# ishine/zerovox.cpp

Hardware: AMD Instinct MI355X
Metric: audio-seconds/wall-second (xRT) end-to-end phoneme->22.05 kHz wav (higher is better)
Workload: dtype f16*f16->f32 (MFMA) convs, f32 (MFMA) attention/linear, f32 activations

## Files before the change

### zerovox.cpp_amd/csrc/capi.cpp

```cpp
#include <algorithm>
#include <cmath>
#include <cstring>
#include <map>
#include <optional>
#include <string>
#include <thread>
#include <vector>

#include "common.h"
#include "model.h"
#include "knobs.h"

using zv::Model;

struct PendingBatch;
struct zv_model
{
    Model        *m;
    PendingBatch *pending;
};

static void free_pending(zv_model *m);
static void lane0_select(zv_model *m);
static void use_lane0(zv_model *m);
// ... 278 lines not shown
static zv_status run_single(zv_model *m, const Request &r, std::optional<Taps> taps = std::nullopt)
{
    return guarded([&] {
        check_request(m, r);
        Model &M = *m->m;
        use_lane0(m);
        const uint32_t n = r.n[0], T = r.T[0];
        const bool tg = r.targets(), pc = r.phoneme_controls() || tg, dur = r.timings();
        const size_t E = M.E(), b_ids = (size_t)n * 4, b_hid = (size_t)T * E * 4, b_wav = (size_t)T * M.hp.audio_hop_size * 4;
        const size_t b_ctl = r.prosody || tg ? zv::CTL_STRIDE * 4 : 0, b_pctl = pc ? (size_t)n * zv::PCTL_STRIDE * 4 : 0;
        if (!taps) M.reserve(n, T);
        Layout L;
        const size_t o_nf = L.at(4), o_ids = L.at(b_ids), o_pun = L.at(b_ids), o_sty = L.at(E * 4), o_ctl = L.at(b_ctl),
                     o_pctl = L.at(b_pctl), o_hid = L.at(b_hid);
        const size_t o_mel = taps ? 0 : L.at((size_t)T * M.hp.audio_num_mels * 4), o_wav = taps ? 0 : L.at(b_wav),
                     o_cum = taps ? 0 : L.at(dur ? b_ids : 0), o_live = L.at(r.fitted && !taps ? sizeof(zv::Seg) : 0);
        char *io = (char *)M.io_scratch(L.size());
        int32_t *d_nf = (int32_t *)(io + o_nf), *d_ids = (int32_t *)(io + o_ids), *d_pun = (int32_t *)(io + o_pun);
        float *d_sty = (float *)(io + o_sty), *d_hid = (float *)(io + o_hid);
        std::vector<float> ctl(b_ctl / 4), pctl(b_pctl / 4);
        std::vector<int32_t> cum(dur ? n : 0);
        pack_controls(r, ctl.data(), pctl.data());
        zv::Batch bt = zv::Batch::single(n, T, r.num_phonemes[0]);
        bt.has_targets = tg;
        ZV_HIP(hipMemcpyAsync(d_ids, r.ids[0], b_ids, hipMemcpyHostToDevice, M.stream()));
        ZV_HIP(hipMemcpyAsync(d_pun, r.puncts[0], b_ids, hipMemcpyHostToDevice, M.stream()));
        ZV_HIP(hipMemcpyAsync(d_sty, r.styles[0], E * 4, hipMemcpyHostToDevice, M.stream()));
        if (b_ctl)
        {
            bt.d_ctl = (const float *)(io + o_ctl);
            ZV_HIP(hipMemcpyAsync(io + o_ctl, ctl.data(), b_ctl, hipMemcpyHostToDevice, M.stream()));
        }
        if (b_pctl)
        {
            bt.d_pctl = (const float *)(io + o_pctl);
            ZV_HIP(hipMemcpyAsync(io + o_pctl, pctl.data(), b_pctl, hipMemcpyHostToDevice, M.stream()));
        }
        int32_t nf = 0;
        if (taps)
// ... 1 lines not shown
            const Model::EncoderTaps t = M.encode_dev(bt, d_ids, d_pun, d_sty, d_hid, d_nf);
            ZV_HIP(hipMemcpyAsync(r.out[0], d_hid, b_hid, hipMemcpyDeviceToHost, M.stream()));
            ZV_HIP(hipMemcpyAsync(&nf, d_nf, 4, hipMemcpyDeviceToHost, M.stream()));
            if (taps->features) ZV_HIP(hipMemcpyAsync(taps->features, t.features, (size_t)n * E * 4, hipMemcpyDeviceToHost, M.stream()));
            if (taps->logdur) ZV_HIP(hipMemcpyAsync(taps->logdur, t.logdur, b_ids, hipMemcpyDeviceToHost, M.stream()));
            if (taps->pitch) ZV_HIP(hipMemcpyAsync(taps->pitch, t.pitch, b_ids, hipMemcpyDeviceToHost, M.stream()));
            if (taps->energy) ZV_HIP(hipMemcpyAsync(taps->energy, t.energy, b_ids, hipMemcpyDeviceToHost, M.stream()));
            if (taps->pitch_bucket) ZV_HIP(hipMemcpyAsync(taps->pitch_bucket, t.pitch_bucket, b_ids, hipMemcpyDeviceToHost, M.stream()));
            if (taps->energy_bucket) ZV_HIP(hipMemcpyAsync(taps->energy_bucket, t.energy_bucket, b_ids, hipMemcpyDeviceToHost, M.stream()));
            if (dur) ZV_HIP(hipMemcpyAsync(cum.data(), t.cum, b_ids, hipMemcpyDeviceToHost, M.stream()));
        }
        else
        {
            float *d_mel = (float *)(io + o_mel), *d_wav = (float *)(io + o_wav);
            if (dur) bt.d_cum = (int32_t *)(io + o_cum);
            if (r.fitted) bt.d_frm_live = (zv::Seg *)(io + o_live);
            M.chain_dev(bt, d_ids, d_pun, d_sty, d_hid, d_mel, d_wav, d_nf);
            ZV_HIP(hipMemcpyAsync(&nf, d_nf, 4, hipMemcpyDeviceToHost, M.stream()));
            if (dur) ZV_HIP(hipMemcpyAsync(cum.data(), bt.d_cum, b_ids, hipMemcpyDeviceToHost, M.stream()));
            ZV_HIP(hipMemcpyAsync(r.out[0], d_wav, b_wav, hipMemcpyDeviceToHost, M.stream()));
        }
        M.sync();
        if (r.n_frames) r.n_frames[0] = (uint32_t)nf;
        if (dur) durations_from_cum(cum.data(), 1, r.n, r.T, r.durations);
    });
}

zv_status zv_encode_taps(zv_model *m, const int32_t *ids, const int32_t *puncts, const float *style, uint32_t n,
                         uint32_t num_phonemes, uint32_t T, float *hidden, uint32_t *n_frames, float *features, float *logdur,
                         float *pitch, float *energy, int32_t *pitch_bucket, int32_t *energy_bucket)
{
// ... 223 lines not shown
    zv::Batch bt;
    bt.nseg = (int)r.count;
    bt.n_max = zv::round_up((int)nmax, 32);
    bt.n_real = (int)nmax;
    bt.t_max = zv::round_up((int)tmax, 64);
    bt.n_rows = (size_t)bt.nseg * bt.n_max;
    bt.t_rows = (size_t)bt.nseg * bt.t_max;
    Layout in;
    const size_t b_tab = (size_t)(bt.nseg + 1) * sizeof(zv::Seg);
    const size_t i_tok = in.at(b_tab), i_frm = in.at(b_tab), i_ids = in.at(bt.n_rows * 4), i_pun = in.at(bt.n_rows * 4),
                 i_sty = in.at((size_t)bt.nseg * E * 4), i_ctl = in.at(ctl ? (size_t)bt.nseg * zv::CTL_STRIDE * 4 : 0),
                 i_pctl = in.at(pc ? bt.n_rows * zv::PCTL_STRIDE * 4 : 0), b_in = in.size();
    Layout dev;
    const size_t o_nf = dev.at((size_t)bt.nseg * 4), o_in = dev.at(b_in), o_hid = dev.at(bt.t_rows * E * 4),
                 o_mel = dev.at(bt.t_rows * Mm * 4), o_wav = dev.at(bt.t_rows * hop * 4), o_cum = dev.at(dur ? bt.n_rows * 4 : 0),
                 o_live = dev.at(r.fitted ? (size_t)bt.nseg * sizeof(zv::Seg) : 0);
    M.reserve_batch(bt);
    char *io = (char *)M.io_scratch(dev.size());
    size_t wav_bytes = 0;
    pb.woff.assign(r.count, 0);
    for (uint32_t u = 0; u < r.count; u++)
    {
        pb.woff[u] = wav_bytes;
        wav_bytes += (size_t)r.T[u] * hop * 4;
    }
    Layout host;
    const size_t p_in = host.at(b_in), p_nf = host.at((size_t)bt.nseg * 4), p_wav = host.at(wav_bytes),
                 p_cum = host.at(dur ? bt.n_rows * 4 : 0);
    char *pin = (char *)M.pinned_scratch(host.size());
    char *d_in = io + o_in, *h_in = pin + p_in;
    {
// ... 11 lines not shown
            memcpy(h_sty + (size_t)u * E, r.styles[u], E * 4);
            n0 += n;
            t0 += t;
        }
        h_tok[r.count] = zv::Seg{0, n0, n0, 0};
        h_frm[r.count] = zv::Seg{0, t0, 0, 0};
        pack_controls(r, (float *)(h_in + i_ctl), (float *)(h_in + i_pctl));
    }
    bt.d_tok = (const zv::Seg *)(d_in + i_tok);
    bt.d_frm = (const zv::Seg *)(d_in + i_frm);
    if (ctl) bt.d_ctl = (const float *)(d_in + i_ctl);
    bt.has_targets = tg;
    if (pc) bt.d_pctl = (const float *)(d_in + i_pctl);
    if (dur) bt.d_cum = (int32_t *)(io + o_cum);
    if (r.fitted) bt.d_frm_live = (zv::Seg *)(io + o_live);
    int32_t *d_nf = (int32_t *)(io + o_nf), *d_ids = (int32_t *)(d_in + i_ids), *d_pun = (int32_t *)(d_in + i_pun);
    float *d_sty = (float *)(d_in + i_sty), *d_hid = (float *)(io + o_hid), *d_mel = (float *)(io + o_mel), *d_wav = (float *)(io + o_wav);
    int32_t *h_nf = (int32_t *)(pin + p_nf), *h_cum = dur ? (int32_t *)(pin + p_cum) : nullptr;
    char *h_wav = pin + p_wav;
    const int G = (M.tail_groups() > 1 && bt.nseg >= 4 && wav_bytes >= ((size_t)16 << 20) && !M.profiling && M.dbg_layer.kind < 0)
                      ? std::min(M.tail_groups(), (int)bt.nseg / 2) : 1;
    try
    {
        hipStream_t cs = M.copy_stream();
        pb.gb.assign(G + 1, r.count);
        pb.gb[0] = 0;
        const uint64_t seq = M.next_batch_seq();
        ZV_HIP(hipEventRecord(M.batch_event(seq, 0), M.stream()));
        if (G <= 1)
        {
// ... 605 lines not shown
```

### zerovox.cpp_amd/csrc/decoder.cpp

```cpp
#include "schedule.h"

#include <cmath>

namespace zv
{

Model::DecLayout Model::dec_layout(DeviceArena &a, const Batch &bt) const
{
    const size_t S = (size_t)bt.nseg, L = bt.t_rows, B = 2 * E(), R = (size_t)dec_.R, CAT = B + R;
    DecLayout d{(bt.t_max + 31) / 32, round_up(dec_.fc_out + 64, 64), 2 * (int)CAT + 64};
    d.h = a.take_n<float>(S * d.hs);
    for (float **st : {&d.st_x, &d.st_t, &d.st_y, &d.st_a}) *st = a.take_n<float>(S * d.ss);
    for (double **p : {&d.part_t, &d.part_o}) *p = a.take_n<double>(S * d.nblk * CAT * 2);
    d.cat = a.take_n<float>(L * CAT);
    for (float **x : {&d.t1, &d.sc, &d.x0, &d.xa}) *x = a.take_n<float>(L * B);
    d.asr_t = a.take_n<float>(L * R);
    d.xa16 = a.take_n<_Float16>(L * CAT);
    d.t16 = a.take_n<_Float16>(L * B);
    d.xr16 = a.take_n<_Float16>(L * CAT);
    return d;
}

void Model::decode_dev(const Batch &bt, const float *d_hidden, const float *d_styles, float *d_mel)
{
    if (bt.t_rows == 0 || bt.t_max <= 0) fail(ZV_ERR_ARG, "T must be > 0");
    const DecLayout lay = dec_layout(stage_arena(bt), bt);
    const Segs fr = bt.frames();
    const int Ed = (int)E(), B = 2 * Ed, R = dec_.R, CAT = B + R, S = bt.nseg;
    const size_t L = bt.t_rows;
    const int nblk = lay.nblk, hs = lay.hs, ss = lay.ss;
    float *const h = lay.h, *const st_x = lay.st_x, *const st_t = lay.st_t, *const st_y = lay.st_y, *const st_a = lay.st_a;
    double *const part_t = lay.part_t, *const part_o = lay.part_o;
    float *const cat = lay.cat, *const t1 = lay.t1, *const sc = lay.sc, *const x0 = lay.x0, *const xa = lay.xa, *const asr_t = lay.asr_t;
    _Float16 *const xa16 = lay.xa16, *const t16 = lay.t16, *const xr16 = lay.xr16;
    const double Ld = (double)L;
    const int pre_env = knob(ZV_DEC_PREPASS);
    const bool prepass = pre_env >= 0 ? pre_env != 0 : (size_t)bt.t_max * bt.nseg >= 256;

    ZV_LAUNCH("dec_adain_fc", 4.0 * dec_.fc_out * (Ed + 2), 2.0 * S * dec_.fc_out * Ed,
              launch_linear(stream(), d_styles, Ed, Ed, dec_.fcW, dec_.fcB, dec_.fc_out, h, hs, dec_.fcExtra, segs_single(S)));

    const float rsqrt2 = (float)(1.0 / sqrt(2.0));

    auto finalize = [&](const double *part, int C, float *stat, int c_off) {
        ZV_LAUNCH("dec_in_stats", 16.0 * S * nblk * C, 4.0 * S * nblk * C,
                  launch_stats_finalize(stream(), part, nblk, C, 1e-5f, stat, ss, c_off, fr, 1));
    };
    auto norm_input = [&](ConvJob &j, const float *x, int ldx, int C, const double *part, int Cpart, float *stat, const float *g,
                          const float *b, int gb_seg, _Float16 *op16, _Float16 *raw16 = nullptr) {
        if (prepass)
        {
            ZV_LAUNCH("dec_norm_operand", 6.0 * Ld * C, 8.0 * Ld * C,
                      launch_norm_act_f16(stream(), x, ldx, C, part, nblk, Cpart, 1e-5f, stat, ss, g, b, gb_seg, 0.2f, op16, C, fr, raw16));
            j.x0 = op16;
            j.ldx = C;
            j.pro = PRO_RAW_F16;
        }
        else
        {
            finalize(part, Cpart, stat, 0);
            j.x0 = x;
            j.ldx = ldx;
            j.pro = PRO_NORM_ACT;
            j.pstat = stat;
            j.pstat_seg = ss;
            j.pa = g;
            j.pb = b;
            j.pab_seg = gb_seg;
// ... 119 lines not shown
    const int ldos[5] = {CAT, CAT, Ed, Ed, Ed};
    const int cparts[5] = {B, B, B, Ed, Ed};
    float *sts[5] = {st_x, st_x, st_x, st_y, st_y};
    for (int i = 0; i < 5; i++)
    {
        const DecBlk &b = dec_.dec[i];
        block(b, cur, ldc, cparts[i], sts[i], h + b.g1, h + b.g1 + b.cin, h + b.g2, h + b.g2 + b.cout, hs, outs[i], ldos[i], i < 4);
        cur = outs[i];
        ldc = ldos[i];
    }
    if (dbg_layer.done) return;
    {
        ConvJob j = job(dec_.to_out);
        j.x0 = cur;
        j.ldx = ldc;
        j.out = d_mel;
        j.ldo = dec_.M;
        if (dbg_layer.kind == ZV_LAYER_DEC_TO_OUT) dbg_inject(const_cast<float *>(cur), ldc, Ed, L);
        conv(&j, 1, fr, 1, "dec_conv", conv_bytes(Ld, Ed, dec_.M, 1, false), conv_flops(Ld, Ed, dec_.M, 1));
        if (dbg_layer.kind == ZV_LAYER_DEC_TO_OUT) dbg_extract(d_mel, dec_.M, dec_.M, L);
    }
}

}
```

### zerovox.cpp_amd/csrc/encoder.cpp

```cpp
#include "schedule.h"

#include <cmath>

namespace zv
{

Model::EncLayout Model::enc_layout(DeviceArena &a, const Batch &bt) const
{
    const size_t n = bt.n_rows, Ed = E();
    EncLayout e{round_up(enc_.dur.V, 16)};
    for (float **p : {&e.x, &e.y}) *p = a.take_n<float>(n * Ed);
    e.qkv = a.take_n<float>(n * 3 * Ed);
    for (float **p : {&e.o, &e.f}) *p = a.take_n<float>(n * Ed);
    e.hh = a.take_n<_Float16>(n * round_up(hp.conv_filter_size, 16));
    for (float **p : {&e.va, &e.vb}) *p = a.take_n<float>(n * e.Vp);
    for (float **p : {&e.t.logdur, &e.t.pitch, &e.t.energy}) *p = a.take_n<float>(n);
    for (int32_t **p : {&e.t.pitch_bucket, &e.t.energy_bucket}) *p = a.take_n<int32_t>(n);
    e.t.cum = bt.d_cum ? bt.d_cum : a.take_n<int32_t>(n);
    e.t.features = e.x;
    return e;
}

Model::EncoderTaps Model::encode_dev(const Batch &bt, const int32_t *d_ids, const int32_t *d_puncts, const float *d_styles,
                                     float *d_hidden, int32_t *d_nframes)
// ... 113 lines not shown
    };
    predictor(enc_.dur, t.logdur, nullptr, nullptr, 0, 0);
    predictor(enc_.pitch, t.pitch, enc_.pitch_emb, t.pitch_bucket, CTL_PITCH, PCTL_PITCH);
    if (dbg_layer.done) return t;
    predictor(enc_.energy, t.energy, enc_.energy_emb, t.energy_bucket, CTL_ENERGY, PCTL_ENERGY);
    if (dbg_layer.done) return t;
    if (bt.has_targets)
    {
        if (!bt.d_ctl || !bt.d_pctl) fail(ZV_ERR_ARG, "a batch with target durations needs its control rows");
        ZV_LAUNCH("enc_fit_durations", 24.0 * nd, 0.0, launch_fit_durations(stream(), t.logdur, bt.d_ctl, bt.d_pctl, tk, fr));
    }
    ZV_LAUNCH("enc_length_regulator", 4.0 * (nd + (double)bt.t_rows) * Ed, 0.0,
              launch_length_regulator(stream(), x, Ed, t.logdur, Ed, d_hidden, Ed, t.cum, d_nframes, tk, fr, bt.d_ctl, bt.d_pctl));
    if (bt.d_frm_live)
        ZV_LAUNCH("enc_live_frames", 36.0 * bt.nseg, 0.0, launch_live_frames(stream(), d_nframes, bt.d_frm_live, fr));
    return t;
}

void Model::debug_layernorm(int index, uint32_t n)
{
    const int l = index >> 1, Ed = (int)E();
    if (index < 0 || l >= (int)enc_.layers.size()) return;
    const EncLayer &Ly = enc_.layers[l];
    float *d = (float *)io_scratch(2 * (size_t)n * Ed * 4), *y = d + (size_t)n * Ed;
    dbg_inject(d, Ed, Ed, n);
    ZV_HIP(launch_add_layernorm(stream(), d, Ed, nullptr, 0, Ed, Ed, (index & 1) ? Ly.ln2w : Ly.ln1w, (index & 1) ? Ly.ln2b : Ly.ln1b,
                                1e-5f, y, Ed, segs_single((int)n)));
    dbg_extract(y, Ed, Ed, n);
}

// ... 2 lines not shown
```

### zerovox.cpp_amd/csrc/kernels.h

```cpp
#pragma once

#include <hip/hip_runtime.h>
#include <stdint.h>

#ifdef ZV_DIAG
#define ZV_DBGBITS(x) (x)
#else
#define ZV_DBGBITS(x) 0
#endif

namespace zv
{

__host__ __device__ static inline int round_up(int x, int a) { return (x + a - 1) / a * a; }

struct Seg
{
    int32_t row0, rows;
    int32_t aux;
    int32_t pad;
};
struct Segs
{
    const Seg *tab;
// ... 161 lines not shown
{
    const float *x0, *x1, *x2;
    int          ldx, L, C, K;
    float        pscale, slope;
    const uint16_t *w;
    float        bias;
    float       *out;
    Segs         segs;
    int          rate;
    int          runs;
};
hipError_t launch_out_conv(hipStream_t s, const OutConvArgs &a);

hipError_t launch_stats_partial(hipStream_t s, const float *x, int ldx, int C, double *part, int nblk, const Segs &segs, int rate);
hipError_t launch_stats_finalize(hipStream_t s, const double *part, int nblk, int C, float eps, float *stat, int stat_seg,
                                 int c_off, const Segs &segs, int rate);
hipError_t launch_norm_apply(hipStream_t s, const float *x, int ldx, int C, const float *stat, int stat_seg, const float *g,
                             const float *b, float *y, int ldy, double *part, int nblk, const Segs &segs);

hipError_t launch_act_f16(hipStream_t s, const float *x0, const float *x1, const float *x2, float pscale, float slope, void *out, size_t n);
hipError_t launch_norm_act_f16(hipStream_t s, const float *x, int ldx, int C, const double *part, int nblk, int Cpart, float eps,
                               float *stat, int stat_seg, const float *ga, const float *be, int gb_seg, float slope, void *y,
                               int ldy, const Segs &segs, void *yraw = nullptr);

hipError_t launch_linear(hipStream_t s, const float *x, int ldx, int in, const float *W, const float *b, int out, float *y,
                         int ldy, const float *extra, const Segs &segs);

hipError_t launch_embed(hipStream_t s, const int32_t *ids, const int32_t *puncts, const float *wemb, int emb,
                        const float *pemb, int pdim, const float *posenc, float *x, int ld, const Segs &segs);
hipError_t launch_attention(hipStream_t s, const float *q, const float *k, const float *v, int ld, int H, int dk,
                            float inv_temp, float *o, int ldo, const Segs &segs);
constexpr int CTL_STRIDE = 8;
constexpr int CTL_DURATION = 0;
constexpr int CTL_PITCH = 1;
constexpr int CTL_ENERGY = 3;
constexpr int CTL_TARGET = 5;
constexpr int PCTL_STRIDE = 4;
constexpr int PCTL_FRAMES = 0;
// ... 17 lines not shown
hipError_t launch_length_regulator(hipStream_t s, const float *feat, int ld, const float *logdur, int C, float *hidden,
                                   int ldh, int32_t *cum, int32_t *n_frames, const Segs &tokens, const Segs &frames,
                                   const float *ctl = nullptr, const float *pctl = nullptr);

constexpr int FIT_MAX_TOKENS = 3584;
hipError_t launch_fit_durations(hipStream_t s, const float *logdur, const float *ctl, const float *pctl, const Segs &tokens,
                                const Segs &frames);

hipError_t launch_live_frames(hipStream_t s, const int32_t *n_frames, Seg *live, const Segs &frames);
hipError_t launch_zero_tail(hipStream_t s, float *x, int C, const Segs &frames, const Segs &live, int rate);

constexpr int VOC_RUN_MARGIN = 16;
hipError_t launch_voc_runs(hipStream_t s, const float *mel, int M, float *mel_c, int32_t *eq, Seg *runs, const Segs &frames, int H);
hipError_t launch_voc_run_fill(hipStream_t s, float *x, const Segs &runs, int rate);

}
```

### zerovox.cpp_amd/csrc/knobs.h

```cpp
#pragma once

namespace zv
{

#define ZV_KNOB_LIST(X)                                                                                                               \
    X(ZV_NO_FUSE, 0)                                                                  \
    X(ZV_NO_TRIPLE, 0)                                                                          \
    X(ZV_FUSE256, 0)                                                \
    X(ZV_NO_MERGE, 0)                                                               \
    X(ZV_MERGE_ALWAYS, 0)                 \
    X(ZV_MERGE_SEQ, 1)          \
    X(ZV_MERGE_MAXC, 256)                                  \
    X(ZV_TAIL_GROUPS, 8)                                                        \
    X(ZV_ARENA_FILL, 0)                                         \
    X(ZV_DEC_PREPASS, -1)                                      \
    X(ZV_CONV_MT, 0)                                                              \
    X(ZV_CONV_NT, 0)                                                     \
    X(ZV_CONV_SINGLE, 1)                                    \
    X(ZV_CONV_GEMM, 1)                  \
    X(ZV_CONV_STREAM, 1)        \
    X(ZV_VOC_RUNS, 1)           \
    X(ZV_UP_GEMM, 1)            \
    X(ZV_GEMM_ORDER, 2)         \
    X(ZV_PAIR_MT, 0)                                                                  \
    X(ZV_CONV_XCD, 1)           \
    X(ZV_CONV_WARM, 1)          \
    X(ZV_LINEAR_MERGED, 1)      \
    X(ZV_BLOCK64, 3)            \
    X(ZV_PAIR64_RING, 1)               \
    X(ZV_TRIPLE_V2, 1)                               \
    X(ZV_TRIPLE_DB, 1)                                                                     \
    X(ZV_TRIPLE_INTERLEAVE, 1)                                                               \
    X(ZV_ATT_SCALAR, 0)                                                                               \
    X(ZV_ATT_MFMA, 0)                                                          \
    X(ZV_LN_TAIL, 1)

// ... 34 lines not shown
```

### zerovox.cpp_amd/csrc/misc_kernels.hip

```cpp
#include "kernels.h"
#include "knobs.h"
#include "fit_durations.h"

#include <cstring>

namespace zv
{

__device__ __forceinline__ double wave_sum(double v)
{
#pragma unroll
    for (int o = 32; o > 0; o >>= 1) v += __shfl_xor(v, o, 64);
    return v;
}
__device__ __forceinline__ float wave_sum_f(float v)
{
#pragma unroll
    for (int o = 32; o > 0; o >>= 1) v += __shfl_xor(v, o, 64);
    return v;
}

typedef float floatx16m __attribute__((ext_vector_type(16)));

__global__ __launch_bounds__(256) void stats_partial_kernel(const float *__restrict__ x, int ldx, int C,
// ... 24 lines not shown
    {
        const double a = (red[0][0][cl] + red[0][1][cl]) + (red[0][2][cl] + red[0][3][cl]);
        const double b = (red[1][0][cl] + red[1][1][cl]) + (red[1][2][cl] + red[1][3][cl]);
        *(double2 *)(part + (((size_t)useg * nblk + blk) * C + c) * 2) = make_double2(a, b);
    }
}

hipError_t launch_stats_partial(hipStream_t s, const float *x, int ldx, int C, double *part, int nblk, const Segs &segs, int rate)
{
    const int nb = (segs.max_rows * rate + 31) / 32;
    if (nb > nblk || segs.nseg < 1) return hipErrorInvalidValue;
    hipLaunchKernelGGL(stats_partial_kernel, dim3((C + 63) / 64, nb, segs.nseg), dim3(256), 0, s, x, ldx, C, part, nblk, segs, rate);
    return hipGetLastError();
}

__device__ __forceinline__ float2 stats_from_partials(const double *__restrict__ p, int C, int nb, int L, float eps)
{
    double s1 = 0.0, s2 = 0.0;
    for (int b0 = 0; b0 < nb; b0 += 8)
    {
        double2 v[8];
#pragma unroll
        for (int i = 0; i < 8; i++) v[i] = *(const double2 *)(p + (size_t)(b0 + i < nb ? b0 + i : nb - 1) * C * 2);
#pragma unroll
        for (int i = 0; i < 8; i++)
            if (b0 + i < nb)
            {
                s1 += v[i].x;
                s2 += v[i].y;
            }
    }
    const double mean = s1 / (double)L;
    double var = s2 / (double)L - mean * mean;
    var = var > 0.0 ? var : 0.0;
    return make_float2((float)mean, 1.0f / sqrtf((float)var + eps));
}

__global__ __launch_bounds__(64) void stats_finalize_kernel(const double *__restrict__ part, int nblk, int C, float eps,
                                                            float *__restrict__ stat, int stat_seg, int c_off,
                                                            const Segs segs, int rate)
{
    const int useg = blockIdx.y;
    const Seg sg = seg_at(segs, useg);
    const int L = sg.rows * rate;
    const int c = blockIdx.x * 64 + threadIdx.x;
    if (c >= C || L <= 0) return;
    const float2 mr = stats_from_partials(part + ((size_t)useg * nblk * C + c) * 2, C, (L + 31) >> 5, L, eps);
    float *o = stat + (size_t)useg * stat_seg + 2 * (c_off + c);
    o[0] = mr.x;
    o[1] = mr.y;
}

hipError_t launch_stats_finalize(hipStream_t s, const double *part, int nblk, int C, float eps, float *stat, int stat_seg,
                                 int c_off, const Segs &segs, int rate)
{
    if (segs.nseg < 1) return hipErrorInvalidValue;
    hipLaunchKernelGGL(stats_finalize_kernel, dim3((C + 63) / 64, segs.nseg), dim3(64), 0, s, part, nblk, C, eps, stat, stat_seg,
                       c_off, segs, rate);
    return hipGetLastError();
}

__global__ __launch_bounds__(256) void norm_apply_kernel(const float *__restrict__ x, int ldx, int C,
                                                         const float *__restrict__ stat, int stat_seg,
                                                         const float *__restrict__ g, const float *__restrict__ b,
                                                         float *__restrict__ y, int ldy, double *__restrict__ part, int nblk,
                                                         const Segs segs)
{
    __shared__ double red[2][4][64];
    const int useg = blockIdx.z, blk = blockIdx.y;
    const Seg sg = seg_at(segs, useg);
    const int L = sg.rows;
    if (blk * 32 >= L) return;
    const int cl = threadIdx.x & 63, rg = threadIdx.x >> 6;
// ... 35 lines not shown
hipError_t launch_norm_apply(hipStream_t s, const float *x, int ldx, int C, const float *stat, int stat_seg, const float *g,
                             const float *b, float *y, int ldy, double *part, int nblk, const Segs &segs)
{
    const int nb = (segs.max_rows + 31) / 32;
    if ((part && nb > nblk) || segs.nseg < 1) return hipErrorInvalidValue;
    hipLaunchKernelGGL(norm_apply_kernel, dim3((C + 63) / 64, nb, segs.nseg), dim3(256), 0, s, x, ldx, C, stat, stat_seg, g, b, y,
                       ldy, part, nblk, segs);
    return hipGetLastError();
}

__global__ __launch_bounds__(256) void norm_act_f16_kernel(const float *__restrict__ x, int ldx, int C,
                                                           const double *__restrict__ part, int nblk, int Cpart, float eps,
                                                           float *__restrict__ stat, int stat_seg,
                                                           const float *__restrict__ ga, const float *__restrict__ be, int gb_seg,
                                                           float slope, _Float16 *__restrict__ y, int ldy, _Float16 *__restrict__ yraw,
                                                           const Segs segs)
{
    __shared__ float sm[4][64];
    const int useg = blockIdx.y;
    const Seg sg = seg_at(segs, useg);
    const int L = sg.rows;
    if (L <= 0) return;
    const int tid = threadIdx.x;
    if (tid < 64)
    {
        const int c = blockIdx.x * 64 + tid;
        float2 mr = make_float2(0.f, 0.f);
        float g = 0.f, b = 0.f;
        if (c < C)
        {
            float *st = stat + (size_t)useg * stat_seg + 2 * c;
            if (c < Cpart)
            {
                mr = stats_from_partials(part + ((size_t)useg * nblk * Cpart + c) * 2, Cpart, (L + 31) >> 5, L, eps);
                st[0] = mr.x;
                st[1] = mr.y;
            }
            else
                mr = make_float2(st[0], st[1]);
            g = ga[(size_t)useg * gb_seg + c];
            b = be[(size_t)useg * gb_seg + c];
        }
        sm[0][tid] = mr.x;
        sm[1][tid] = mr.y;
        sm[2][tid] = g;
        sm[3][tid] = b;
    }
    __syncthreads();
    const int c4 = (tid & 15) * 4, rl = tid >> 4;
// ... 33 lines not shown
            if (yr)
            {
                half4v hr;
                hr[0] = (_Float16)v[u].x;
                hr[1] = (_Float16)v[u].y;
                hr[2] = (_Float16)v[u].z;
                hr[3] = (_Float16)v[u].w;
                *(half4v *)(yr + (size_t)t * ldy) = hr;
            }
        }
    }
}

hipError_t launch_norm_act_f16(hipStream_t s, const float *x, int ldx, int C, const double *part, int nblk, int Cpart, float eps,
                               float *stat, int stat_seg, const float *ga, const float *be, int gb_seg, float slope, void *y,
                               int ldy, const Segs &segs, void *yraw)
{
    if ((C & 3) || (ldx & 3) || (ldy & 3) || segs.nseg < 1 || Cpart > C) return hipErrorInvalidValue;
    if (Cpart > 0 && (segs.max_rows + 31) / 32 > nblk) return hipErrorInvalidValue;
    int gz = 1;
    while (gz < 8 && (long)((C + 63) / 64) * segs.nseg * gz < 2048 && gz * 128 < segs.max_rows) gz <<= 1;
    hipLaunchKernelGGL(norm_act_f16_kernel, dim3((C + 63) / 64, segs.nseg, gz), dim3(256), 0, s, x, ldx, C, part, nblk, Cpart, eps, stat,
                       stat_seg, ga, be, gb_seg, slope, (_Float16 *)y, ldy, (_Float16 *)yraw, segs);
    return hipGetLastError();
}

typedef _Float16 half4v __attribute__((ext_vector_type(4)));
__global__ __launch_bounds__(256) void act_f16_kernel(const float4 *__restrict__ x0, const float4 *__restrict__ x1,
                                                      const float4 *__restrict__ x2, float pscale, float slope,
                                                      half4v *__restrict__ out, size_t n4)
{
    const size_t stride = (size_t)gridDim.x * 256;
    for (size_t i0 = (size_t)blockIdx.x * 256 + threadIdx.x; i0 < n4; i0 += 4 * stride)
    {
        float4 v[4], a[4], b[4];
#pragma unroll
        for (int u = 0; u < 4; u++)
        {
// ... 1248 lines not shown
    for (int k = 0; k < 4; k++)
    {
        const long i = i0 + k * 256 + threadIdx.x;
        if (i < n) dst[i] = src[i % rate];
    }
}

hipError_t launch_voc_run_fill(hipStream_t s, float *x, const Segs &runs, int rate)
{
    if (runs.nseg < 1 || runs.max_rows < 1 || rate < 1 || !runs.tab || !x) return hipErrorInvalidValue;
    const long per_seg = (long)runs.max_rows * rate;
    hipLaunchKernelGGL(voc_run_fill_kernel, dim3((unsigned)((per_seg + 1023) / 1024), runs.nseg), dim3(256), 0, s, x, runs.tab, rate);
    return hipGetLastError();
}

}
```

### zerovox.cpp_amd/csrc/model.h

```cpp
#pragma once

#include <cstdint>
#include <cstring>
#include <string>
#include <vector>

#include "common.h"
#include "gguf_reader.h"
#include "kernels.h"

namespace zv
{

struct ConvW
{
    void  *w = nullptr;
    void  *w8 = nullptr;
    float *bias = nullptr;
    int    K = 0, Cin = 0, Cout = 0, Cin_p = 0, Cout_p = 0, ck = 0;
};

struct DeviceArena
{
    char  *base = nullptr;
// ... 18 lines not shown
    int         launches;
};

struct Batch
{
    int        nseg = 1;
    int        n_max = 0, t_max = 0;
    int        n_real = 0;
    size_t     n_rows = 0, t_rows = 0;
    const Seg *d_tok = nullptr, *d_frm = nullptr;
    Seg        tok1{0, 0, 0, 0}, frm1{0, 0, 0, 0};
    const float *d_ctl = nullptr;
    const float *d_pctl = nullptr;
    int32_t *d_cum = nullptr;
    Seg *d_frm_live = nullptr;
    bool has_targets = false;

    static Batch single(uint32_t N, uint32_t T, uint32_t num_phonemes)
    {
        Batch b;
        b.n_max = (int)N;
        b.n_real = (int)N;
        b.t_max = (int)T;
        b.n_rows = N;
        b.t_rows = T;
        b.tok1 = Seg{0, (int32_t)N, (int32_t)num_phonemes, 0};
        b.frm1 = Seg{0, (int32_t)T, 0, 0};
        return b;
    }
    Segs tokens() const { return Segs{d_tok, nseg, n_max, tok1}; }
    Segs tokens_merged() const { return d_tok ? Segs{d_tok + nseg, 1, (int)n_rows, tok1} : tokens(); }
    Segs frames_cap() const { return Segs{d_frm, nseg, t_max, frm1}; }
    Segs frames() const { return d_frm_live ? Segs{d_frm_live, nseg, t_max, frm1} : frames_cap(); }
    bool same_schedule(const Batch &o) const
    {
        return nseg == o.nseg && n_max == o.n_max && t_max == o.t_max && n_rows == o.n_rows && t_rows == o.t_rows && d_tok == o.d_tok &&
               d_frm == o.d_frm && (d_tok || memcmp(&tok1, &o.tok1, sizeof(Seg)) == 0) && (d_frm || memcmp(&frm1, &o.frm1, sizeof(Seg)) == 0) &&
               d_ctl == o.d_ctl && d_pctl == o.d_pctl && d_cum == o.d_cum && d_frm_live == o.d_frm_live && has_targets == o.has_targets;
    }
};

struct CapturedGraph
{
    static constexpr int NKEY = 8;
    int            kind = 0;
    unsigned       epoch = 0;
    Batch          b;
    const void    *p[NKEY] = {};
    hipGraphExec_t exec = nullptr;
    const Seg     *runs_tab = nullptr;
    int            runs_n = 0;
};

// ... 35 lines not shown
        bool         done = false;
    } dbg_layer;

    uint32_t max_phonemes() const { return (uint32_t)enc_.posenc_rows; }
    void reserve(uint32_t max_phonemes, uint32_t max_frames);
    void reserve_batch(const Batch &b);
    int  voc_stage_rate(int stage) const;
    int  voc_stage_channels(int stage) const;
    uint32_t max_frames_per_utterance() const;
    int wemb_rows() const { return enc_.wemb_rows; }
    int pemb_rows() const { return enc_.pemb_rows; }
    uint32_t vocoder_halo_frames() const;
    bool voc_runs_off = false;
    bool voc_runs_on(const Batch &b) const;
    const Seg *voc_runs_last(int *n) { *n = lane().runs_n; return lane().runs_tab; }
    void sync();

    void select_lane(int i);
    int  selected_lane() const { return cur_lane_; }
    void sync_all_lanes();
    void poison_lane(int i, int byte, size_t filled[3]);

    void *io_scratch(size_t bytes);
    void *pinned_scratch(size_t bytes);

    bool graph_mode = false;
    void vocode_dev_graph(const Batch &b, const float *d_mel, float *d_wav);
    void chain_dev(const Batch &b, const int32_t *d_ids, const int32_t *d_puncts, const float *d_styles, float *d_hidden,
                   float *d_mel, float *d_wav, int32_t *d_nframes, const void *h2d_src = nullptr, void *h2d_dst = nullptr,
                   size_t h2d_bytes = 0, int voc_part = 0);
// ... 66 lines not shown
        std::vector<EncLayer> layers;
        VarPred dur, pitch, energy;
    } enc_;

    struct VocLayout
    {
        float *c0;
        struct Stage { float *ub, *y[3]; _Float16 *xt[3]; } st[8];
        float *mel_c; int32_t *eq; Seg *runs;
    };
    struct DecLayout
    {
        int    nblk, hs, ss;
        float *h, *st_x, *st_t, *st_y, *st_a, *cat, *t1, *sc, *x0, *xa, *asr_t;
        double *part_t, *part_o; _Float16 *xa16, *t16, *xr16;
    };
    struct EncLayout { int Vp; float *x, *y, *qkv, *o, *f, *va, *vb; _Float16 *hh; EncoderTaps t; };
    VocLayout voc_layout(DeviceArena &a, const Batch &b) const;
    DecLayout dec_layout(DeviceArena &a, const Batch &b) const;
    EncLayout enc_layout(DeviceArena &a, const Batch &b) const;
    static constexpr size_t ARENA_TAIL = (size_t)1 << 20;
    size_t arena_bytes_for(const Batch &b) const;
    void  arena_require(size_t bytes);
    DeviceArena &stage_arena(const Batch &b);

    void conv(const ConvJob *jobs, int n, const Segs &segs, int rate, const char *name, double bytes, double flops);
    void dbg_inject(void *dev, int ld, int cols, size_t rows);
    void dbg_extract(const void *dev, int ld, int cols, size_t rows);
    ConvJob job(const ConvW &w) const;
    void tick(hipEvent_t *e0);
// ... 40 lines not shown
```

Before: 31530.

## Skip decoder work on padded frame tail via compacted run table

Adds a per-segment decoder run table, computed after the length regulator, that drops 32-row blocks of padding beyond each utterance's real frames plus the decoder receptive-field reach. The decoder convs and norms then run on the compacted rows. Instance-norm statistics are corrected by counting the block at the gap boundary G extra times, and the output mel is expanded back to the full layout. This removes decoder compute on padded frames for large batches, at the cost of an extra expand kernel and a layout buffer. It also relies on the replicated-block statistics matching what the full-length run would give.

```diff
diff --git a/zerovox.cpp_amd/csrc/capi.cpp b/zerovox.cpp_amd/csrc/capi.cpp
--- a/zerovox.cpp_amd/csrc/capi.cpp
+++ b/zerovox.cpp_amd/csrc/capi.cpp
@@ -316,7 +316,8 @@
         const size_t o_nf = L.at(4), o_ids = L.at(b_ids), o_pun = L.at(b_ids), o_sty = L.at(E * 4), o_ctl = L.at(b_ctl),
                      o_pctl = L.at(b_pctl), o_hid = L.at(b_hid);
         const size_t o_mel = taps ? 0 : L.at((size_t)T * M.hp.audio_num_mels * 4), o_wav = taps ? 0 : L.at(b_wav),
-                     o_cum = taps ? 0 : L.at(dur ? b_ids : 0), o_live = L.at(r.fitted && !taps ? sizeof(zv::Seg) : 0);
+                     o_cum = taps ? 0 : L.at(dur ? b_ids : 0), o_live = L.at(r.fitted && !taps ? sizeof(zv::Seg) : 0),
+                     o_runs = L.at(!r.fitted && !taps ? sizeof(zv::Seg) : 0);
         char *io = (char *)M.io_scratch(L.size());
         int32_t *d_nf = (int32_t *)(io + o_nf), *d_ids = (int32_t *)(io + o_ids), *d_pun = (int32_t *)(io + o_pun);
         float *d_sty = (float *)(io + o_sty), *d_hid = (float *)(io + o_hid);
@@ -325,6 +326,8 @@
         pack_controls(r, ctl.data(), pctl.data());
         zv::Batch bt = zv::Batch::single(n, T, r.num_phonemes[0]);
         bt.has_targets = tg;
+        if (r.fitted && !taps) bt.d_frm_live = (zv::Seg *)(io + o_live);
+        if (!taps && M.dec_runs_on(bt)) bt.d_dec_runs = (zv::Seg *)(io + o_runs);
         ZV_HIP(hipMemcpyAsync(d_ids, r.ids[0], b_ids, hipMemcpyHostToDevice, M.stream()));
         ZV_HIP(hipMemcpyAsync(d_pun, r.puncts[0], b_ids, hipMemcpyHostToDevice, M.stream()));
         ZV_HIP(hipMemcpyAsync(d_sty, r.styles[0], E * 4, hipMemcpyHostToDevice, M.stream()));
@@ -356,7 +359,6 @@
         {
             float *d_mel = (float *)(io + o_mel), *d_wav = (float *)(io + o_wav);
             if (dur) bt.d_cum = (int32_t *)(io + o_cum);
-            if (r.fitted) bt.d_frm_live = (zv::Seg *)(io + o_live);
             M.chain_dev(bt, d_ids, d_pun, d_sty, d_hid, d_mel, d_wav, d_nf);
             ZV_HIP(hipMemcpyAsync(&nf, d_nf, 4, hipMemcpyDeviceToHost, M.stream()));
             if (dur) ZV_HIP(hipMemcpyAsync(cum.data(), bt.d_cum, b_ids, hipMemcpyDeviceToHost, M.stream()));
@@ -610,7 +612,8 @@
     Layout dev;
     const size_t o_nf = dev.at((size_t)bt.nseg * 4), o_in = dev.at(b_in), o_hid = dev.at(bt.t_rows * E * 4),
                  o_mel = dev.at(bt.t_rows * Mm * 4), o_wav = dev.at(bt.t_rows * hop * 4), o_cum = dev.at(dur ? bt.n_rows * 4 : 0),
-                 o_live = dev.at(r.fitted ? (size_t)bt.nseg * sizeof(zv::Seg) : 0);
+                 o_live = dev.at(r.fitted ? (size_t)bt.nseg * sizeof(zv::Seg) : 0),
+                 o_runs = dev.at(!r.fitted ? (size_t)bt.nseg * sizeof(zv::Seg) : 0);
     M.reserve_batch(bt);
     char *io = (char *)M.io_scratch(dev.size());
     size_t wav_bytes = 0;
@@ -652,6 +655,7 @@
     if (pc) bt.d_pctl = (const float *)(d_in + i_pctl);
     if (dur) bt.d_cum = (int32_t *)(io + o_cum);
     if (r.fitted) bt.d_frm_live = (zv::Seg *)(io + o_live);
+    if (M.dec_runs_on(bt)) bt.d_dec_runs = (zv::Seg *)(io + o_runs);
     int32_t *d_nf = (int32_t *)(io + o_nf), *d_ids = (int32_t *)(d_in + i_ids), *d_pun = (int32_t *)(d_in + i_pun);
     float *d_sty = (float *)(d_in + i_sty), *d_hid = (float *)(io + o_hid), *d_mel = (float *)(io + o_mel), *d_wav = (float *)(io + o_wav);
     int32_t *h_nf = (int32_t *)(pin + p_nf), *h_cum = dur ? (int32_t *)(pin + p_cum) : nullptr;
diff --git a/zerovox.cpp_amd/csrc/dec_runs.h b/zerovox.cpp_amd/csrc/dec_runs.h
--- /dev/null
+++ b/zerovox.cpp_amd/csrc/dec_runs.h
@@ -0,0 +1,78 @@
+#pragma once
+
+#include <stddef.h>
+
+#if defined(__HIPCC__)
+#define ZV_DR_FN __host__ __device__ static inline
+#else
+#define ZV_DR_FN static inline
+#endif
+
+namespace zv
+{
+
+constexpr int DEC_RUN_BLOCK = 32;
+constexpr int DEC_RUN_MARGIN = 32;
+
+struct DecRun
+{
+    int rows_c;
+    int gap_at;
+    int G;
+};
+
+ZV_DR_FN DecRun dec_run(int n, int T, int R)
+{
+    const DecRun whole = {T, 0, 0};
+    n = n < 0 ? 0 : (n < T ? n : T);
+    if (R < 0 || T - R - 1 < 0) return whole;
+    const long a = ((long)n + R + 2 * DEC_RUN_BLOCK - 1) / DEC_RUN_BLOCK * DEC_RUN_BLOCK;
+    const long b = (long)(T - R - 1) / DEC_RUN_BLOCK * DEC_RUN_BLOCK;
+    if (b - a < DEC_RUN_BLOCK || b - a < DEC_RUN_MARGIN) return whole;
+    const DecRun r = {(int)(a + (T - b)), (int)(a / DEC_RUN_BLOCK), (int)((b - a) / DEC_RUN_BLOCK)};
+    return r;
+}
+
+ZV_DR_FN int dec_run_compact_row(int t, int gap_at, int G)
+{
+    const int a = gap_at * DEC_RUN_BLOCK, b = a + G * DEC_RUN_BLOCK;
+    return (G <= 0 || t < a) ? t : (t < b ? a - 1 : t - G * DEC_RUN_BLOCK);
+}
+ZV_DR_FN int dec_run_original_row(int c, int gap_at, int G) { return (G <= 0 || c < gap_at * DEC_RUN_BLOCK) ? c : c + G * DEC_RUN_BLOCK; }
+
+ZV_DR_FN void dec_run_block_sum(const double *p, size_t stride, int nb, int gap_at, int G, double *sum, double *sumsq)
+{
+    double s1 = 0.0, s2 = 0.0;
+    for (int b0 = 0; b0 < nb; b0 += 8)
+    {
+        double v1[8], v2[8];
+#if defined(__HIPCC__)
+#pragma unroll
+#endif
+        for (int i = 0; i < 8; i++)
+        {
+            const double *q = p + (size_t)(b0 + i < nb ? b0 + i : nb - 1) * stride;
+            v1[i] = q[0];
+            v2[i] = q[1];
+        }
+#if defined(__HIPCC__)
+#pragma unroll
+#endif
+        for (int i = 0; i < 8; i++)
+            if (b0 + i < nb)
+            {
+                s1 += v1[i];
+                s2 += v2[i];
+                if (b0 + i + 1 == gap_at)
+                    for (int k = 0; k < G; k++)
+                    {
+                        s1 += v1[i];
+                        s2 += v2[i];
+                    }
+            }
+    }
+    *sum = s1;
+    *sumsq = s2;
+}
+
+}
diff --git a/zerovox.cpp_amd/csrc/decoder.cpp b/zerovox.cpp_amd/csrc/decoder.cpp
--- a/zerovox.cpp_amd/csrc/decoder.cpp
+++ b/zerovox.cpp_amd/csrc/decoder.cpp
@@ -1,5 +1,6 @@
 #include "schedule.h"
 
+#include <algorithm>
 #include <cmath>
 
 namespace zv
@@ -18,14 +19,38 @@
     d.xa16 = a.take_n<_Float16>(L * CAT);
     d.t16 = a.take_n<_Float16>(L * B);
     d.xr16 = a.take_n<_Float16>(L * CAT);
+    d.mel_c = a.take_n<float>(L * dec_.M);
     return d;
+}
+
+bool Model::dec_prepass_on(const Batch &bt) const
+{
+    const int pre_env = knob(ZV_DEC_PREPASS);
+    return pre_env >= 0 ? pre_env != 0 : (size_t)bt.t_max * bt.nseg >= 256;
+}
+
+bool Model::dec_runs_on(const Batch &bt) const
+{
+    const int k = knob(ZV_DEC_RUNS);
+    return k != 0 && !bt.d_frm_live && dbg_layer.kind < 0 && dec_prepass_on(bt) && (k == 2 || (long)bt.t_rows >= 16384);
+}
+
+int Model::dec_reach_frames() const
+{
+    auto half = [](const ConvW &w) { return w.K > 0 ? (w.K - 1) / 2 : 0; };
+    auto blk = [&](const DecBlk &b) { return std::max(half(b.conv1) + half(b.conv2), b.learned_sc ? half(b.sc) : 0); };
+    int r = std::max(blk(dec_.enc[0]) + blk(dec_.enc[1]), half(dec_.asr0));
+    for (const DecBlk &b : dec_.dec) r += blk(b);
+    return r + half(dec_.to_out);
 }
 
 void Model::decode_dev(const Batch &bt, const float *d_hidden, const float *d_styles, float *d_mel)
 {
     if (bt.t_rows == 0 || bt.t_max <= 0) fail(ZV_ERR_ARG, "T must be > 0");
     const DecLayout lay = dec_layout(stage_arena(bt), bt);
-    const Segs fr = bt.frames();
+    const bool runs = bt.d_dec_runs != nullptr;
+    if (runs && !dec_runs_on(bt)) fail(ZV_ERR_ARG, "internal: a decoder run table on a schedule that takes none");
+    const Segs fr = runs ? Segs{bt.d_dec_runs, bt.nseg, bt.t_max, bt.frm1} : bt.frames();
     const int Ed = (int)E(), B = 2 * Ed, R = dec_.R, CAT = B + R, S = bt.nseg;
     const size_t L = bt.t_rows;
     const int nblk = lay.nblk, hs = lay.hs, ss = lay.ss;
@@ -33,9 +58,16 @@
     double *const part_t = lay.part_t, *const part_o = lay.part_o;
     float *const cat = lay.cat, *const t1 = lay.t1, *const sc = lay.sc, *const x0 = lay.x0, *const xa = lay.xa, *const asr_t = lay.asr_t;
     _Float16 *const xa16 = lay.xa16, *const t16 = lay.t16, *const xr16 = lay.xr16;
-    const double Ld = (double)L;
-    const int pre_env = knob(ZV_DEC_PREPASS);
-    const bool prepass = pre_env >= 0 ? pre_env != 0 : (size_t)bt.t_max * bt.nseg >= 256;
+    double Ld = (double)L;
+    if (runs && profiling)
+    {
+        std::vector<Seg> tab((size_t)S);
+        ZV_HIP(hipMemcpyAsync(tab.data(), bt.d_dec_runs, tab.size() * sizeof(Seg), hipMemcpyDeviceToHost, stream()));
+        ZV_HIP(hipStreamSynchronize(stream()));
+        Ld = 0;
+        for (const Seg &g : tab) Ld += g.rows;
+    }
+    const bool prepass = dec_prepass_on(bt);
 
     ZV_LAUNCH("dec_adain_fc", 4.0 * dec_.fc_out * (Ed + 2), 2.0 * S * dec_.fc_out * Ed,
               launch_linear(stream(), d_styles, Ed, Ed, dec_.fcW, dec_.fcB, dec_.fc_out, h, hs, dec_.fcExtra, segs_single(S)));
@@ -44,14 +76,14 @@
 
     auto finalize = [&](const double *part, int C, float *stat, int c_off) {
         ZV_LAUNCH("dec_in_stats", 16.0 * S * nblk * C, 4.0 * S * nblk * C,
-                  launch_stats_finalize(stream(), part, nblk, C, 1e-5f, stat, ss, c_off, fr, 1));
+                  launch_stats_finalize(stream(), part, nblk, C, 1e-5f, stat, ss, c_off, fr, 1, runs));
     };
     auto norm_input = [&](ConvJob &j, const float *x, int ldx, int C, const double *part, int Cpart, float *stat, const float *g,
                           const float *b, int gb_seg, _Float16 *op16, _Float16 *raw16 = nullptr) {
         if (prepass)
         {
             ZV_LAUNCH("dec_norm_operand", 6.0 * Ld * C, 8.0 * Ld * C,
-                      launch_norm_act_f16(stream(), x, ldx, C, part, nblk, Cpart, 1e-5f, stat, ss, g, b, gb_seg, 0.2f, op16, C, fr, raw16));
+                      launch_norm_act_f16(stream(), x, ldx, C, part, nblk, Cpart, 1e-5f, stat, ss, g, b, gb_seg, 0.2f, op16, C, fr, raw16, runs));
             j.x0 = op16;
             j.ldx = C;
             j.pro = PRO_RAW_F16;
@@ -201,12 +233,15 @@
         ConvJob j = job(dec_.to_out);
         j.x0 = cur;
         j.ldx = ldc;
-        j.out = d_mel;
+        j.out = runs ? lay.mel_c : d_mel;
         j.ldo = dec_.M;
         if (dbg_layer.kind == ZV_LAYER_DEC_TO_OUT) dbg_inject(const_cast<float *>(cur), ldc, Ed, L);
         conv(&j, 1, fr, 1, "dec_conv", conv_bytes(Ld, Ed, dec_.M, 1, false), conv_flops(Ld, Ed, dec_.M, 1));
         if (dbg_layer.kind == ZV_LAYER_DEC_TO_OUT) dbg_extract(d_mel, dec_.M, dec_.M, L);
     }
-}
-
-}
+    if (runs)
+        ZV_LAUNCH("dec_run_expand", 4.0 * (Ld + (double)L) * dec_.M, 0.0,
+                  launch_dec_run_expand(stream(), lay.mel_c, d_mel, dec_.M, fr, bt.frames_cap()));
+}
+
+}
diff --git a/zerovox.cpp_amd/csrc/encoder.cpp b/zerovox.cpp_amd/csrc/encoder.cpp
--- a/zerovox.cpp_amd/csrc/encoder.cpp
+++ b/zerovox.cpp_amd/csrc/encoder.cpp
@@ -151,6 +151,8 @@
               launch_length_regulator(stream(), x, Ed, t.logdur, Ed, d_hidden, Ed, t.cum, d_nframes, tk, fr, bt.d_ctl, bt.d_pctl));
     if (bt.d_frm_live)
         ZV_LAUNCH("enc_live_frames", 36.0 * bt.nseg, 0.0, launch_live_frames(stream(), d_nframes, bt.d_frm_live, fr));
+    if (bt.d_dec_runs)
+        ZV_LAUNCH("enc_dec_runs", 36.0 * bt.nseg, 0.0, launch_dec_runs(stream(), d_nframes, bt.d_dec_runs, fr, dec_reach_frames()));
     return t;
 }
 
diff --git a/zerovox.cpp_amd/csrc/kernels.h b/zerovox.cpp_amd/csrc/kernels.h
--- a/zerovox.cpp_amd/csrc/kernels.h
+++ b/zerovox.cpp_amd/csrc/kernels.h
@@ -199,14 +199,14 @@
 
 hipError_t launch_stats_partial(hipStream_t s, const float *x, int ldx, int C, double *part, int nblk, const Segs &segs, int rate);
 hipError_t launch_stats_finalize(hipStream_t s, const double *part, int nblk, int C, float eps, float *stat, int stat_seg,
-                                 int c_off, const Segs &segs, int rate);
+                                 int c_off, const Segs &segs, int rate, int dec_runs = 0);
 hipError_t launch_norm_apply(hipStream_t s, const float *x, int ldx, int C, const float *stat, int stat_seg, const float *g,
                              const float *b, float *y, int ldy, double *part, int nblk, const Segs &segs);
 
 hipError_t launch_act_f16(hipStream_t s, const float *x0, const float *x1, const float *x2, float pscale, float slope, void *out, size_t n);
 hipError_t launch_norm_act_f16(hipStream_t s, const float *x, int ldx, int C, const double *part, int nblk, int Cpart, float eps,
                                float *stat, int stat_seg, const float *ga, const float *be, int gb_seg, float slope, void *y,
-                               int ldy, const Segs &segs, void *yraw = nullptr);
+                               int ldy, const Segs &segs, void *yraw = nullptr, int dec_runs = 0);
 
 hipError_t launch_linear(hipStream_t s, const float *x, int ldx, int in, const float *W, const float *b, int out, float *y,
                          int ldy, const float *extra, const Segs &segs);
@@ -254,4 +254,7 @@
 hipError_t launch_voc_runs(hipStream_t s, const float *mel, int M, float *mel_c, int32_t *eq, Seg *runs, const Segs &frames, int H);
 hipError_t launch_voc_run_fill(hipStream_t s, float *x, const Segs &runs, int rate);
 
+hipError_t launch_dec_runs(hipStream_t s, const int32_t *n_frames, Seg *runs, const Segs &frames, int R);
+hipError_t launch_dec_run_expand(hipStream_t s, const float *mel_c, float *mel, int M, const Segs &runs, const Segs &frames);
+
 }
diff --git a/zerovox.cpp_amd/csrc/knobs.h b/zerovox.cpp_amd/csrc/knobs.h
--- a/zerovox.cpp_amd/csrc/knobs.h
+++ b/zerovox.cpp_amd/csrc/knobs.h
@@ -20,6 +20,7 @@
     X(ZV_CONV_GEMM, 1)                  \
     X(ZV_CONV_STREAM, 1)        \
     X(ZV_VOC_RUNS, 1)           \
+    X(ZV_DEC_RUNS, 1)           \
     X(ZV_UP_GEMM, 1)            \
     X(ZV_GEMM_ORDER, 2)         \
     X(ZV_PAIR_MT, 0)                                                                  \
diff --git a/zerovox.cpp_amd/csrc/misc_kernels.hip b/zerovox.cpp_amd/csrc/misc_kernels.hip
--- a/zerovox.cpp_amd/csrc/misc_kernels.hip
+++ b/zerovox.cpp_amd/csrc/misc_kernels.hip
@@ -1,6 +1,7 @@
 #include "kernels.h"
 #include "knobs.h"
 #include "fit_durations.h"
+#include "dec_runs.h"
 
 #include <cstring>
 
@@ -62,49 +63,44 @@
     return hipGetLastError();
 }
 
-__device__ __forceinline__ float2 stats_from_partials(const double *__restrict__ p, int C, int nb, int L, float eps)
-{
-    double s1 = 0.0, s2 = 0.0;
-    for (int b0 = 0; b0 < nb; b0 += 8)
-    {
-        double2 v[8];
-#pragma unroll
-        for (int i = 0; i < 8; i++) v[i] = *(const double2 *)(p + (size_t)(b0 + i < nb ? b0 + i : nb - 1) * C * 2);
-#pragma unroll
-        for (int i = 0; i < 8; i++)
-            if (b0 + i < nb)
-            {
-                s1 += v[i].x;
-                s2 += v[i].y;
-            }
-    }
+__device__ __forceinline__ float2 stats_from_partials(const double *__restrict__ p, int C, int nb, int L, float eps, int gap_at = 0, int G = 0)
+{
+    double s1, s2;
+    dec_run_block_sum(p, (size_t)C * 2, nb, gap_at, G, &s1, &s2);
     const double mean = s1 / (double)L;
     double var = s2 / (double)L - mean * mean;
     var = var > 0.0 ? var : 0.0;
     return make_float2((float)mean, 1.0f / sqrtf((float)var + eps));
 }
 
+__device__ __forceinline__ int2 dec_run_gap(const Segs &segs, int useg, int dec_runs)
+{
+    if (!dec_runs || !segs.tab) return make_int2(0, 0);
+    return make_int2(__builtin_amdgcn_readfirstlane(segs.tab[useg].aux), __builtin_amdgcn_readfirstlane(segs.tab[useg].pad));
+}
+
 __global__ __launch_bounds__(64) void stats_finalize_kernel(const double *__restrict__ part, int nblk, int C, float eps,
                                                             float *__restrict__ stat, int stat_seg, int c_off,
-                                                            const Segs segs, int rate)
+                                                            const Segs segs, int rate, int dec_runs)
 {
     const int useg = blockIdx.y;
     const Seg sg = seg_at(segs, useg);
     const int L = sg.rows * rate;
     const int c = blockIdx.x * 64 + threadIdx.x;
     if (c >= C || L <= 0) return;
-    const float2 mr = stats_from_partials(part + ((size_t)useg * nblk * C + c) * 2, C, (L + 31) >> 5, L, eps);
+    const int2 gap = dec_run_gap(segs, useg, dec_runs);
+    const float2 mr = stats_from_partials(part + ((size_t)useg * nblk * C + c) * 2, C, (L + 31) >> 5, L + DEC_RUN_BLOCK * gap.y, eps, gap.x, gap.y);
     float *o = stat + (size_t)useg * stat_seg + 2 * (c_off + c);
     o[0] = mr.x;
     o[1] = mr.y;
 }
 
 hipError_t launch_stats_finalize(hipStream_t s, const double *part, int nblk, int C, float eps, float *stat, int stat_seg,
-                                 int c_off, const Segs &segs, int rate)
-{
-    if (segs.nseg < 1) return hipErrorInvalidValue;
+                                 int c_off, const Segs &segs, int rate, int dec_runs)
+{
+    if (segs.nseg < 1 || (dec_runs && (!segs.tab || rate != 1))) return hipErrorInvalidValue;
     hipLaunchKernelGGL(stats_finalize_kernel, dim3((C + 63) / 64, segs.nseg), dim3(64), 0, s, part, nblk, C, eps, stat, stat_seg,
-                       c_off, segs, rate);
+                       c_off, segs, rate, dec_runs);
     return hipGetLastError();
 }
 
@@ -170,7 +166,7 @@
                                                            float *__restrict__ stat, int stat_seg,
                                                            const float *__restrict__ ga, const float *__restrict__ be, int gb_seg,
                                                            float slope, _Float16 *__restrict__ y, int ldy, _Float16 *__restrict__ yraw,
-                                                           const Segs segs)
+                                                           const Segs segs, int dec_runs)
 {
     __shared__ float sm[4][64];
     const int useg = blockIdx.y;
@@ -188,7 +184,8 @@
             float *st = stat + (size_t)useg * stat_seg + 2 * c;
             if (c < Cpart)
             {
-                mr = stats_from_partials(part + ((size_t)useg * nblk * Cpart + c) * 2, Cpart, (L + 31) >> 5, L, eps);
+                const int2 gap = dec_run_gap(segs, useg, dec_runs);
+                mr = stats_from_partials(part + ((size_t)useg * nblk * Cpart + c) * 2, Cpart, (L + 31) >> 5, L + DEC_RUN_BLOCK * gap.y, eps, gap.x, gap.y);
                 st[0] = mr.x;
                 st[1] = mr.y;
             }
@@ -252,14 +249,14 @@
 
 hipError_t launch_norm_act_f16(hipStream_t s, const float *x, int ldx, int C, const double *part, int nblk, int Cpart, float eps,
                                float *stat, int stat_seg, const float *ga, const float *be, int gb_seg, float slope, void *y,
-                               int ldy, const Segs &segs, void *yraw)
-{
-    if ((C & 3) || (ldx & 3) || (ldy & 3) || segs.nseg < 1 || Cpart > C) return hipErrorInvalidValue;
+                               int ldy, const Segs &segs, void *yraw, int dec_runs)
+{
+    if ((C & 3) || (ldx & 3) || (ldy & 3) || segs.nseg < 1 || Cpart > C || (dec_runs && !segs.tab)) return hipErrorInvalidValue;
     if (Cpart > 0 && (segs.max_rows + 31) / 32 > nblk) return hipErrorInvalidValue;
     int gz = 1;
     while (gz < 8 && (long)((C + 63) / 64) * segs.nseg * gz < 2048 && gz * 128 < segs.max_rows) gz <<= 1;
     hipLaunchKernelGGL(norm_act_f16_kernel, dim3((C + 63) / 64, segs.nseg, gz), dim3(256), 0, s, x, ldx, C, part, nblk, Cpart, eps, stat,
-                       stat_seg, ga, be, gb_seg, slope, (_Float16 *)y, ldy, (_Float16 *)yraw, segs);
+                       stat_seg, ga, be, gb_seg, slope, (_Float16 *)y, ldy, (_Float16 *)yraw, segs, dec_runs);
     return hipGetLastError();
 }
 
@@ -1538,4 +1535,48 @@
     return hipGetLastError();
 }
 
-}
+__global__ __launch_bounds__(64) void dec_runs_kernel(const int32_t *__restrict__ n_frames, Seg *__restrict__ runs, const Segs frames, int R)
+{
+    const int u = blockIdx.x * 64 + threadIdx.x;
+    if (u >= frames.nseg) return;
+    const Seg cap = frames.tab ? frames.tab[u] : frames.one;
+    const DecRun r = dec_run(n_frames[u], cap.rows, R);
+    *(int4 *)(runs + u) = make_int4(cap.row0, r.rows_c, r.gap_at, r.G);
+}
+
+hipError_t launch_dec_runs(hipStream_t s, const int32_t *n_frames, Seg *runs, const Segs &frames, int R)
+{
+    if (frames.nseg < 1 || !n_frames || !runs || R < 0 || (!frames.tab && frames.nseg != 1)) return hipErrorInvalidValue;
+    hipLaunchKernelGGL(dec_runs_kernel, dim3((frames.nseg + 63) / 64), dim3(64), 0, s, n_frames, runs, frames, R);
+    return hipGetLastError();
+}
+
+__global__ __launch_bounds__(256) void dec_run_expand_kernel(const float *__restrict__ src, float *__restrict__ dst, int M,
+                                                             const Seg *__restrict__ runs, const Segs frames)
+{
+    const Seg cap = seg_at(frames, blockIdx.y);
+    const int4 e = *(const int4 *)(runs + blockIdx.y);
+    const int rows_c = __builtin_amdgcn_readfirstlane(e.y), gap_at = __builtin_amdgcn_readfirstlane(e.z), G = __builtin_amdgcn_readfirstlane(e.w);
+    const long n = (long)cap.rows * M;
+    const size_t base = (size_t)cap.row0 * M;
+#pragma unroll
+    for (int k = 0; k < 4; k++)
+    {
+        const long i = (long)blockIdx.x * 1024 + k * 256 + threadIdx.x;
+        if (i >= n) continue;
+        const int t = (int)(i / M), c = (int)(i - (long)t * M);
+        const int tc = dec_run_compact_row(t, gap_at, G);
+        if (tc < rows_c) dst[base + i] = src[base + (size_t)tc * M + c];
+    }
+}
+
+hipError_t launch_dec_run_expand(hipStream_t s, const float *mel_c, float *mel, int M, const Segs &runs, const Segs &frames)
+{
+    if (frames.nseg < 1 || frames.nseg != runs.nseg || frames.max_rows < 1 || M < 1 || !runs.tab || !mel_c || !mel) return hipErrorInvalidValue;
+    const long per_seg = (long)frames.max_rows * M;
+    hipLaunchKernelGGL(dec_run_expand_kernel, dim3((unsigned)((per_seg + 1023) / 1024), frames.nseg), dim3(256), 0, s, mel_c, mel, M,
+                       runs.tab, frames);
+    return hipGetLastError();
+}
+
+}
diff --git a/zerovox.cpp_amd/csrc/model.h b/zerovox.cpp_amd/csrc/model.h
--- a/zerovox.cpp_amd/csrc/model.h
+++ b/zerovox.cpp_amd/csrc/model.h
@@ -56,6 +56,7 @@
     const float *d_pctl = nullptr;
     int32_t *d_cum = nullptr;
     Seg *d_frm_live = nullptr;
+    Seg *d_dec_runs = nullptr;
     bool has_targets = false;
 
     static Batch single(uint32_t N, uint32_t T, uint32_t num_phonemes)
@@ -78,7 +79,8 @@
     {
         return nseg == o.nseg && n_max == o.n_max && t_max == o.t_max && n_rows == o.n_rows && t_rows == o.t_rows && d_tok == o.d_tok &&
                d_frm == o.d_frm && (d_tok || memcmp(&tok1, &o.tok1, sizeof(Seg)) == 0) && (d_frm || memcmp(&frm1, &o.frm1, sizeof(Seg)) == 0) &&
-               d_ctl == o.d_ctl && d_pctl == o.d_pctl && d_cum == o.d_cum && d_frm_live == o.d_frm_live && has_targets == o.has_targets;
+               d_ctl == o.d_ctl && d_pctl == o.d_pctl && d_cum == o.d_cum && d_frm_live == o.d_frm_live && has_targets == o.has_targets &&
+               d_dec_runs == o.d_dec_runs;
     }
 };
 
@@ -144,6 +146,9 @@
     bool voc_runs_off = false;
     bool voc_runs_on(const Batch &b) const;
     const Seg *voc_runs_last(int *n) { *n = lane().runs_n; return lane().runs_tab; }
+    bool dec_runs_on(const Batch &b) const;
+    bool dec_prepass_on(const Batch &b) const;
+    int  dec_reach_frames() const;
     void sync();
 
     void select_lane(int i);
@@ -240,6 +245,7 @@
         int    nblk, hs, ss;
         float *h, *st_x, *st_t, *st_y, *st_a, *cat, *t1, *sc, *x0, *xa, *asr_t;
         double *part_t, *part_o; _Float16 *xa16, *t16, *xr16;
+        float *mel_c;
     };
     struct EncLayout { int Vp; float *x, *y, *qkv, *o, *f, *va, *vb; _Float16 *hh; EncoderTaps t; };
     VocLayout voc_layout(DeviceArena &a, const Batch &b) const;
```

Result: faster. 32690 (median of 6 runs) (+3.7%).
